# alanqrwang/keymorph

Hardware: AMD Instinct MI355X
Metric: volume-pairs/sec (fwd+bwd) at 256^3, 512 kp, TPS (higher is better)
Workload: dtype f32

## Files before the change

keymorph_amd/csrc/conv_up2.hip:

```cpp
#include <cstdlib>
#include "conv_split.h"

namespace {

constexpr int UX = 32, UY = 4;
constexpr int UHX = UX + 2, UHY = UY + 2, UPL = UHX * UHY * 3;
constexpr int UP_TPB = 512;
constexpr int UP_NST = 32;

template <int TERMS>
__global__ __launch_bounds__(256) void pack_weight_up_kernel(const float* __restrict__ w, __bf16* __restrict__ out,
                                                             int Cout, int Ctot, int cofs, int Cl, int CoutP, int nchunk,
                                                             const float* __restrict__ wscale) {
  const long long total = (long long)nchunk * UP_NST * 2 * CoutP * 8;
  for (long long e = (long long)blockIdx.x * 256 + threadIdx.x; e < total; e += (long long)gridDim.x * 256) {
    const int c = (int)(e & 7);
    long long r = e >> 3;
    const int col = (int)(r % CoutP); r /= CoutP;
    const int h = (int)(r & 1); r >>= 1;
    const int su = (int)(r % UP_NST);
    const int chunk = (int)(r / UP_NST);
    const int ci = chunk * 8 + c, p = su >> 2, st = su & 3;
    const int par[3] = {p >> 2, (p >> 1) & 1, p & 1}, j[3] = {st >> 1, st & 1, h};
    int lo[3], hi[3];
// ... 179 lines not shown
    long long r = e >> 3;
    const int col = (int)(r % CiP); r /= CiP;
    const int h = (int)(r & 1); r >>= 1;
    const int s = (int)(r % DUP_NST);
    const int chunk = (int)(r / DUP_NST);
    const int co = chunk * 8 + c;
    const int idx[3] = {s >> 3, (s >> 1) & 3, 2 * (s & 1) + h};
    int lo[3], hi[3];
#pragma unroll
    for (int a = 0; a < 3; ++a) {
      const int par = (idx[a] + 1) & 1, j = idx[a] <= 1 ? 1 : 0;
      lo[a] = par == 0 ? (j == 0 ? 0 : 1) : (j == 0 ? 0 : 2);
      hi[a] = par == 0 ? (j == 0 ? 0 : 2) : (j == 0 ? 1 : 2);
    }
    float v = 0.f;
    if (co < Cout && col < Cl) {
      const float* wr = w + ((long long)co * Ctot + cofs + col) * 27;
      for (int kz = lo[0]; kz <= hi[0]; ++kz)
        for (int ky = lo[1]; ky <= hi[1]; ++ky)
          for (int kx = lo[2]; kx <= hi[2]; ++kx) v += wr[kz * 9 + ky * 3 + kx];
    }
    float rem = wscale ? v * wscale[0] : v;
#pragma unroll
    for (int t = 0; t < TERMS; ++t) {
      float back;
      const unsigned short hb = to16<TERMS>(rem, back);
      reinterpret_cast<unsigned short*>(out)[((((long long)chunk * TERMS + t) * DUP_NST + s) * 2 + h) * CiP * 8 +
                                             (long long)col * 8 + c] = hb;
      rem -= back;
    }
  }
}

template <int TERMS, bool AMP = false>
__global__ __launch_bounds__(DUP_TPB, TERMS == 2 ? 2 : 3) void conv3_up2_dgrad_kernel(
    const float* __restrict__ dz , const bf16x8* __restrict__ wp,
    float* __restrict__ ds , int Dl, int Hl, int Wl, int Cl, int CiP, int Cout, int tiles_x,
    int tiles_y, const float* __restrict__ dscale, const float* __restrict__ wscale,
    double* __restrict__ stats_partial ,
    int in_blocked ) {
  __shared__ bf16x8 sIn[TERMS][DPL];
  const int tid = threadIdx.x, lane = tid & 63, wv = tid >> 6, li = lane & 31, lh = lane >> 5;
  const int n = blockIdx.z;
  const int ncig = (Cl + 127) / 128;
  const int item = xcd_remap(blockIdx.x, gridDim.x);
  const int cig = item % ncig, brick = item / ncig;
  const int bx = brick % tiles_x, by = (brick / tiles_x) % tiles_y, zl = brick / (tiles_x * tiles_y);
  const int x0 = bx * DUX, y0 = by * DUY;
  const int ci = cig * 128 + 32 * wv + li;
  const int D = 2 * Dl, H = 2 * Hl, W = 2 * Wl;

  f32x16 acc[2];
#pragma unroll
  for (int m = 0; m < 2; ++m)
#pragma unroll
    for (int r = 0; r < 16; ++r) acc[m][r] = 0.f;
  const float sD = dscale ? dscale[0] : 1.f;
  const float desc = (dscale ? dscale[1] : 1.f) * (wscale ? wscale[1] : 1.f);
  const int nchunk = (Cout + KC - 1) / KC;
  const float* dn = dz + (long long)n * D * H * W * Cout;
  constexpr int NV = (DPL + DUP_TPB - 1) / DUP_TPB;
  const int abase = (2 * (li >> 4)) * DHX + 2 * (li & 15) + lh;

  float4 pre[NV][2];
  auto fetch = [&](int ch) {
#pragma unroll
    for (int i = 0; i < NV; ++i) {
      const int v = tid + i * DUP_TPB;
      pre[i][0] = pre[i][1] = make_float4(0.f, 0.f, 0.f, 0.f);
      if (v < DPL) {
        const int lx = v % DHX, ly = (v / DHX) % DHY, lz = v / (DHX * DHY);
        const int gx = 2 * x0 - 1 + lx, gy = 2 * y0 - 1 + ly, gz = 2 * zl - 1 + lz;
        if ((unsigned)gx < (unsigned)W && (unsigned)gy < (unsigned)H && (unsigned)gz < (unsigned)D) {
          const long long vox = ((long long)gz * H + gy) * W + gx;
          const float* p = in_blocked ? dn + ((long long)ch * D * H * W + vox) * KC : dn + vox * Cout + ch * KC;
          if ((Cout & 3) == 0) {
#pragma unroll
            for (int q = 0; q < 2; ++q)
              if (ch * KC + 4 * q < Cout) pre[i][q] = *reinterpret_cast<const float4*>(p + 4 * q);
          } else {
            float t8[8] = {0.f, 0.f, 0.f, 0.f, 0.f, 0.f, 0.f, 0.f};
#pragma unroll
            for (int j = 0; j < 8; ++j)
              if (ch * KC + j < Cout) t8[j] = p[j];
            pre[i][0] = make_float4(t8[0], t8[1], t8[2], t8[3]);
            pre[i][1] = make_float4(t8[4], t8[5], t8[6], t8[7]);
          }
        }
      }
    }
  };
  constexpr bool PF = TERMS == 2;
  if (PF) fetch(0);
  for (int ch = 0; ch < nchunk; ++ch) {
    __syncthreads();
    if (!PF) fetch(ch);
#pragma unroll
    for (int i = 0; i < NV; ++i) {
      const int v = tid + i * DUP_TPB;
      if (v < DPL) {
        const float val[8] = {pre[i][0].x * sD, pre[i][0].y * sD, pre[i][0].z * sD, pre[i][0].w * sD,
                              pre[i][1].x * sD, pre[i][1].y * sD, pre[i][1].z * sD, pre[i][1].w * sD};
        bf16x8 parts[TERMS];
        split8<TERMS>(val, parts);
#pragma unroll
        for (int t = 0; t < TERMS; ++t) sIn[t][v] = parts[t];
      }
    }
    __syncthreads();
    if (PF && ch + 1 < nchunk) fetch(ch + 1);
    const bf16x8* wc = wp + (long long)ch * TERMS * DUP_NST * 2 * CiP + lh * CiP + ci;
    constexpr int BD = 4;
    bf16x8 bq[BD][TERMS];
#pragma unroll
    for (int d = 0; d < BD; ++d)
#pragma unroll
      for (int q = 0; q < TERMS; ++q) bq[d][q] = wc[((long long)(q * DUP_NST + d)) * 2 * CiP];
#pragma unroll 1
    for (int tz = 0; tz < 4; ++tz) {
#pragma unroll
      for (int s8 = 0; s8 < 8; ++s8) {
        const int s = tz * 8 + s8;
        bf16x8 b[TERMS];
#pragma unroll
        for (int q = 0; q < TERMS; ++q) b[q] = bq[s8 % BD][q];
        if (s + BD < DUP_NST) {
#pragma unroll
          for (int q = 0; q < TERMS; ++q) bq[s8 % BD][q] = wc[((long long)(q * DUP_NST + s + BD)) * 2 * CiP];
        }
        const int off = abase + (tz * DHY + (s8 >> 1)) * DHX + 2 * (s8 & 1);
#pragma unroll
        for (int m = 0; m < 2; ++m) {
          bf16x8 a[TERMS];
#pragma unroll
          for (int q = 0; q < TERMS; ++q) a[q] = sIn[q][off + 4 * m * DHX];
          if (TERMS == 3) {
            acc[m] = mfma16<TERMS>(a[2], b[0], acc[m]);
            acc[m] = mfma16<TERMS>(a[1], b[1], acc[m]);
            acc[m] = mfma16<TERMS>(a[0], b[2], acc[m]);
          }
          if constexpr (!AMP) {
            acc[m] = mfma16<TERMS>(a[1], b[0], acc[m]);
            acc[m] = mfma16<TERMS>(a[0], b[1], acc[m]);
          }
          acc[m] = mfma16<TERMS>(a[0], b[0], acc[m]);
        }
      }
    }
  }
  if (ci >= Cl) return;
  float s1 = 0.f, s2 = 0.f;
#pragma unroll
  for (int m = 0; m < 2; ++m) {
#pragma unroll
    for (int r = 0; r < 16; ++r) {
      const int row = (r & 3) + 8 * (r >> 2) + 4 * lh;
      const int gx = x0 + (row & 15), gy = y0 + 2 * m + (row >> 4);
      if (gx < Wl && gy < Hl) {
        const float v = acc[m][r] * desc;
        ds[((((long long)n * Dl + zl) * Hl + gy) * Wl + gx) * Cl + ci] = v;
        s1 += v;
        s2 = fmaf(v, v, s2);
      }
    }
  }
  if (stats_partial) {
    double d1 = (double)s1, d2 = (double)s2;
    d1 += __shfl_xor(d1, 32, 64);
    d2 += __shfl_xor(d2, 32, 64);
    if (lh == 0) {
      double* o = stats_partial + (((long long)n * gridDim.x / ncig + brick) * Cl + ci) * 2;
      o[0] = d1; o[1] = d2;
    }
  }
}

constexpr int GK = 32;
constexpr int GPITCH = GK * 2 + 16;
template <int TERMS, bool AMP = false>
__global__ __launch_bounds__(256, 3) void up2_wgrad_gemm_kernel(const float* __restrict__ A, const float* __restrict__ B,
                                                                float* __restrict__ Cp, int V, int Cl, int J, int kslab,
                                                                int ntn, int ntm, const float* __restrict__ ascale,
                                                                const float* __restrict__ bscale,
                                                                const float* __restrict__ a_scale ,
                                                                const float* __restrict__ a_shift, int xcd) {
  __shared__ __attribute__((aligned(16))) unsigned char sA[TERMS][128 * GPITCH];
  __shared__ __attribute__((aligned(16))) unsigned char sB[TERMS][128 * GPITCH];
  const int tid = threadIdx.x, lane = tid & 63, wv = tid >> 6, li = lane & 31, lh = lane >> 5;
  const int n = blockIdx.z;
  int item = xcd ? xcd_remap((int)blockIdx.x, (int)gridDim.x) : (int)blockIdx.x;
  const int tn = item % ntn; item /= ntn;
  const int tm = item % ntm;
  const int slab = item / ntm;
  const int m0 = tm * 128, n0 = tn * 128;
  const int wm = wv & 1, wn = wv >> 1;
  const float sa = ascale ? ascale[0] : 1.f, sb = bscale ? bscale[0] : 1.f;
  const float desc = (ascale ? ascale[1] : 1.f) * (bscale ? bscale[1] : 1.f);
  const float* An = A + (long long)n * V * Cl;
  const float* Bn = B + (long long)n * V * J;
  f32x16 acc[2][2];
#pragma unroll
  for (int i = 0; i < 2; ++i)
#pragma unroll
    for (int j = 0; j < 2; ++j)
#pragma unroll
// ... 455 lines not shown
  const int xcd = up2_xcd();
  const float* zero16 = (const float*)((const char*)ws + up2_fold_slab_bytes(N, Dl, Hl, Wl, Cl, Cout));
  if (hipMemsetAsync((void*)zero16, 0, 256, s) != hipSuccess) return -12;
  const bool amp = kmh_amp_enabled();
  int rc;
#define KMH_FOLD(A, M) launch_up2_fold<A, M>(g, s, xl, dz, (float*)ws, Dl, Hl, Wl, Cl, Cout, kt, tps, ntm, nto, ascale, dscale, \
                                             a_scale, a_shift, dz_blocked, xcd, zero16)
  if (mode == 2) rc = amp ? KMH_FOLD(true, 2) : KMH_FOLD(false, 2);
  else if (mode == 1) rc = amp ? KMH_FOLD(true, 1) : KMH_FOLD(false, 1);
  else rc = amp ? KMH_FOLD(true, 0) : KMH_FOLD(false, 0);
#undef KMH_FOLD
  if (rc) return rc;
  return up2_reduce(ws, ns, (long long)Cl * 27 * Cout, C, N, s);
}

KMH_API size_t kmh_conv3d_up2_dgrad_pack_bytes(int Cout, int Cl, int terms) {
  const int CiP = (Cl + 127) & ~127;
  return (size_t)((Cout + 7) / 8) * terms * DUP_NST * 2 * CiP * 8 * sizeof(__bf16);
}

KMH_API int kmh_conv3d_up2_dgrad_pack_weight(const float* w, void* packed, int Cout, int Ctot, int cofs, int Cl, int terms,
                                             const float* wscale, void* stream) {
  if (cofs < 0 || cofs + Cl > Ctot || (terms != 2 && terms != 3) || (terms == 2 && !wscale)) return -22;
  const int CiP = (Cl + 127) & ~127, nchunk = (Cout + 7) / 8;
  const long long total = (long long)nchunk * DUP_NST * 2 * CiP * 8;
  int nb = ceil_div(total, 256);
  if (nb > 2048) nb = 2048;
  hipStream_t s = (hipStream_t)stream;
  if (terms == 2) pack_weight_upt_kernel<2><<<nb, 256, 0, s>>>(w, (__bf16*)packed, Cout, Ctot, cofs, Cl, CiP, nchunk, wscale);
  else pack_weight_upt_kernel<3><<<nb, 256, 0, s>>>(w, (__bf16*)packed, Cout, Ctot, cofs, Cl, CiP, nchunk, wscale);
  return KMH_LAUNCH_CHECK();
}

KMH_API size_t kmh_conv3d_up2_dgrad_stats_ws_bytes(int N, int Dl, int Hl, int Wl, int Cl) {
  return (size_t)N * ceil_div(Wl, DUX) * ceil_div(Hl, DUY) * Dl * Cl * 2 * sizeof(double);
}
KMH_API int kmh_conv3d_up2_dgrad(const float* dz, const void* packed, float* ds, int N, int Dl, int Hl, int Wl, int Cl,
                                 int Cout, int terms, const float* dscale, const float* wscale, void* stats_ws,
                                 double* stats_out, int in_blocked, void* stream) {
  KmhAmpCall amp_call(terms);
  if ((terms != 2 && terms != 3) || (terms == 2 && (!dscale || !wscale)) || (stats_out && !stats_ws)) return -22;
  if (in_blocked && (Cout & 7)) return -22;
  const int CiP = (Cl + 127) & ~127;
  const int tx = ceil_div(Wl, DUX), ty = ceil_div(Hl, DUY);
  dim3 g(tx * ty * Dl * ceil_div(Cl, 128), 1, N);
  hipStream_t s = (hipStream_t)stream;
  double* sp = stats_out ? (double*)stats_ws : nullptr;
  if (terms == 2)
    if (kmh_amp_enabled())
      conv3_up2_dgrad_kernel<2, true><<<g, DUP_TPB, 0, s>>>(dz, (const bf16x8*)packed, ds, Dl, Hl, Wl, Cl, CiP, Cout, tx, ty, dscale, wscale, sp, in_blocked);
    else
    conv3_up2_dgrad_kernel<2><<<g, DUP_TPB, 0, s>>>(dz, (const bf16x8*)packed, ds, Dl, Hl, Wl, Cl, CiP, Cout, tx, ty, dscale, wscale, sp, in_blocked);
  else
    conv3_up2_dgrad_kernel<3><<<g, DUP_TPB, 0, s>>>(dz, (const bf16x8*)packed, ds, Dl, Hl, Wl, Cl, CiP, Cout, tx, ty, dscale, wscale, sp, in_blocked);
  if (stats_out)
    kmh_stats::final_kernel<<<dim3(ceil_div(Cl * 2, 256 / kWave), N), 256, 0, s>>>(sp, tx * ty * Dl, Cl, stats_out);
  return KMH_LAUNCH_CHECK();
}

KMH_API size_t kmh_conv3d_up2_pack_bytes(int Cout, int Cl, int terms) {
  return (size_t)(Cl / 8) * terms * UP_NST * 2 * cout_pad(Cout) * 8 * sizeof(__bf16);
}

KMH_API int kmh_conv3d_up2_pack_weight(const float* w, void* packed, int Cout, int Ctot, int cofs, int Cl, int terms,
                                       const float* wscale, void* stream) {
  if ((Cl & 7) || cofs < 0 || cofs + Cl > Ctot || (terms != 2 && terms != 3) || (terms == 2 && !wscale)) return -22;
  const int CoutP = cout_pad(Cout), nchunk = Cl / 8;
  const long long total = (long long)nchunk * UP_NST * 2 * CoutP * 8;
  int nb = ceil_div(total, 256);
  if (nb > 2048) nb = 2048;
  hipStream_t s = (hipStream_t)stream;
  if (terms == 2) pack_weight_up_kernel<2><<<nb, 256, 0, s>>>(w, (__bf16*)packed, Cout, Ctot, cofs, Cl, CoutP, nchunk, wscale);
  else pack_weight_up_kernel<3><<<nb, 256, 0, s>>>(w, (__bf16*)packed, Cout, Ctot, cofs, Cl, CoutP, nchunk, wscale);
  return KMH_LAUNCH_CHECK();
}

KMH_API int kmh_conv3d_up2_fwd(const float* xl, const float* scale, const float* shift, int Ctot, int cofs,
                               const void* packed, float* y, int N, int Dl, int Hl, int Wl, int Cl, int Cout, int terms,
                               const float* ascale, const float* wscale, void* stream) {
  KmhAmpCall amp_call(terms);
  if ((Cl & 7) || (terms != 2 && terms != 3) || (terms == 2 && (!ascale || !wscale))) return -22;
  if ((long long)Dl * Hl * Wl * Cl >= (1ll << 31)) return -22;
  const int CoutP = cout_pad(Cout);
  const int tx = ceil_div(Wl, UX), ty = ceil_div(Hl, UY);
  dim3 g(tx * ty * Dl * ceil_div(Cout, 64), 1, N);
  hipStream_t s = (hipStream_t)stream;
  if (terms == 2)
// ... 12 lines not shown
```

include/keymorph_hip.h:

```cpp
#ifndef KEYMORPH_HIP_H
#define KEYMORPH_HIP_H
#include <stddef.h>
#include <stdint.h>
#ifdef __cplusplus
extern "C" {
#endif

#define KMH_EINVAL (-22)
#define KMH_ABI_VERSION 1
int kmh_abi_version(void);

int kmh_grid_sample3d_fwd(const float* x, const float* grid, float* out, int N, int C, int D, int H,
                          int W, int Do, int Ho, int Wo, int mode, void* stream);
int kmh_grid_sample3d_bwd_grid(const float* x, const float* grid, const float* gout, float* dgrid,
                               int N, int C, int D, int H, int W, int Do, int Ho, int Wo, void* stream);
int kmh_grid_sample3d_bwd_input(const float* grid, const float* gout, float* dx, int N, int C, int D,
                                int H, int W, int Do, int Ho, int Wo, void* stream);

size_t kmh_reduce_ws_bytes(void);
int kmh_mse_fwd(const float* a, const float* b, long long n, float* out, void* ws, void* stream);
int kmh_mse_bwd(const float* a, const float* b, const float* gscale, long long n, float* da, void* stream);
int kmh_warp_mse_fwd(const float* x, const float* grid, const float* fixed, float* out, float* out_loss,
                     int N, int C, int D, int H, int W, int Do, int Ho, int Wo, void* ws, void* stream);
int kmh_warp_mse_fwd_grad(const float* x, const float* grid, const float* fixed, float* out, float* out_loss,
// ... 76 lines not shown
                  void* stream);
int kmh_com3d_bwd(const float* dpts, const float* feat, const float* sums, float* dfeat, int N, int K,
                  int D, int H, int W, void* stream);



int kmh_conv3d_pack_weight(const float* w, float* packed, int Cout, int Cin, int transposed, void* stream);
int kmh_conv3d_fwd(const float* x, const float* scale, const float* shift, const float* mask,
                   const float* packed_w, const float* bias, float* y, int N, int D, int H, int W, int Cin,
                   int Cout, int relu_in, int relu_out, void* stream);
size_t kmh_conv3d_pack_bf_bytes(int Cout, int Cin, int transposed, int terms);
int kmh_conv3d_pack_weight_bf(const float* w, void* packed, int Cout, int Cin, int transposed, int terms,
                              const float* wscale, void* stream);
size_t kmh_conv3d_fwd_bf_stats_ws_bytes(int N, int D, int H, int W, int Cout, int rows_per_wave);
int kmh_conv3d_fwd_bf(const float* x, const float* scale, const float* shift, const float* mask, const void* packed,
                      const float* bias, float* y, int N, int D, int H, int W, int Cin, int Cout, int relu_in,
                      int relu_out, int terms, int rows_per_wave, const float* ascale, const float* wscale,
                      void* stats_ws, double* stats_out, int in_blocked, const float* addend, void* stream);
int kmh_conv3d_fwd_bf_set_dispatch(int mode);
int kmh_conv3d_fwd_bf_split_ok(int N, int D, int H, int W, int Cin, int Cout, int terms);
int kmh_conv3d_fwd_bf_variant(int N, int D, int H, int W, int Cin, int Cout, int terms, int has_mask, int has_addend);
int kmh_conv3d_fwd_bf_pool_ok(int N, int D, int H, int W, int Cin, int Cout, int terms);
int kmh_conv3d_fwd_bf_pool(const float* x, const float* scale, const float* shift, const void* packed, float* yp,
                           unsigned char* arg, int N, int D, int H, int W, int Cin, int Cout, int relu_in, int terms,
                           const float* ascale, const float* wscale, void* stats_ws, double* stats_out, int in_blocked,
                           void* stream);
size_t kmh_conv3d_up2_pack_bytes(int Cout, int Cl, int terms);
int kmh_conv3d_up2_pack_weight(const float* w, void* packed, int Cout, int Ctot, int cofs, int Cl, int terms,
                               const float* wscale, void* stream);
size_t kmh_conv3d_up2_dgrad_pack_bytes(int Cout, int Cl, int terms);
int kmh_conv3d_up2_dgrad_pack_weight(const float* w, void* packed, int Cout, int Ctot, int cofs, int Cl, int terms,
                                     const float* wscale, void* stream);
size_t kmh_conv3d_up2_dgrad_stats_ws_bytes(int N, int Dl, int Hl, int Wl, int Cl);
int kmh_conv3d_up2_dgrad(const float* dz, const void* packed, float* ds, int N, int Dl, int Hl, int Wl, int Cl, int Cout,
                         int terms, const float* dscale, const float* wscale, void* stats_ws, double* stats_out,
                         int in_blocked ,
                         void* stream);
int kmh_up2_boxsum(const float* dz, float* G, int N, int Dl, int Hl, int Wl, int Cout, int in_blocked ,
                   void* stream);
size_t kmh_up2_wgrad_gemm_ws_bytes(int N, int V, int Cl, int J);
int kmh_up2_wgrad_gemm(const float* A, const float* B, float* C, int N, int V, int Cl, int J, int terms,
                       const float* ascale, const float* bscale, const float* a_scale, const float* a_shift, void* ws,
                       void* stream);
int kmh_up2_wgrad_fold_ok(int Cl, int Cout, int terms);
size_t kmh_up2_wgrad_fold_ws_bytes(int N, int Dl, int Hl, int Wl, int Cl, int Cout);
int kmh_up2_wgrad_fold(const float* xl, const float* dz, float* C, int N, int Dl, int Hl, int Wl, int Cl, int Cout, int terms,
                       const float* ascale, const float* dscale, const float* a_scale, const float* a_shift, int dz_blocked,
                       void* ws, void* stream);
int kmh_conv3d_up2_fwd(const float* xl, const float* scale, const float* shift, int Ctot, int cofs, const void* packed,
                       float* y, int N, int Dl, int Hl, int Wl, int Cl, int Cout, int terms, const float* ascale,
                       const float* wscale, void* stream);
size_t kmh_conv3d_wgrad_bf_ws_bytes(int N, int D, int H, int W, int Cin, int Cout, int terms);
int kmh_conv3d_wgrad_bf_blocked_ok(int N, int D, int H, int W, int Cin, int Cout, int terms);
int kmh_conv3d_wgrad_bf(const float* x, const float* scale, const float* shift, const float* dz,
                        const float* dzmask, float* dw, int N, int D, int H, int W, int Cin, int Cout, int relu_in,
                        int accumulate, int terms, int append_ones, const float* xscale, const float* dscale, int dz_blocked, const float* w_fold, double* bhat,
                        void* ws, void* stream);
size_t kmh_conv3d_first_layer_fwd_ws_bytes(int N, int D, int H, int W, int Cout);
int kmh_conv3d_first_layer_fwd(const float* x, const float* scale, const float* shift, const float* w, float* y, int N,
                               int D, int H, int W, int Cout, void* ws, double* stats_out, void* stream);
size_t kmh_conv3d_first_layer_wgrad_ws_bytes(int N, int D, int H, int W, int Cout);
int kmh_conv3d_first_layer_wgrad(const float* x, const float* dz, const float* dzmask, const float* c123, double* rs, int N,
                                 int D, int H, int W, int Cout, void* ws, void* stream);
int kmh_conv3d_first_layer_fold(const void* rs, int rs_f64, const float* w, const float* scale_n, const float* shift_n, int Cout,
                                float* dw, double* ab_n, int accumulate, void* stream);
size_t kmh_conv3d_wgrad_ws_bytes(int N, int D, int H, int W, int Cin, int Cout);
// ... 78 lines not shown
```

keymorph_amd/_lib.py:

```python
from __future__ import annotations

import ctypes as C
import os

from .build import LIBPATH

_f = C.c_void_p
_i = C.c_int
_ll = C.c_longlong
_sz = C.c_size_t

PROTOS = {
    "kmh_abi_version": (_i, []),
    "kmh_grid_sample3d_fwd": (_i, [_f, _f, _f, _i, _i, _i, _i, _i, _i, _i, _i, _i, _f]),
    "kmh_grid_sample3d_bwd_grid": (_i, [_f, _f, _f, _f, _i, _i, _i, _i, _i, _i, _i, _i, _f]),
    "kmh_grid_sample3d_bwd_input": (_i, [_f, _f, _f, _i, _i, _i, _i, _i, _i, _i, _i, _f]),
    "kmh_reduce_ws_bytes": (_sz, []),
    "kmh_mse_fwd": (_i, [_f, _f, _ll, _f, _f, _f]),
    "kmh_mse_bwd": (_i, [_f, _f, _f, _ll, _f, _f]),
    "kmh_warp_mse_fwd": (_i, [_f, _f, _f, _f, _f, _i, _i, _i, _i, _i, _i, _i, _i, _f, _f]),
    "kmh_warp_mse_fwd_grad": (_i, [_f, _f, _f, _f, _f, _f, _i, _i, _i, _i, _i, _i, _i, _i, _f, _f]),
    "kmh_scale_unless_one": (_i, [_f, _ll, _f, _f]),
    "kmh_dice_sums": (_i, [_f, _f, _i, _ll, _f, _f, _f]),
    "kmh_rows_axpby": (_i, [_f, _f, _f, _f, _i, _ll, _f, _f]),
# ... 19 lines not shown
    "kmh_rigid_fit_fwd": (_i, [_f, _f, _f, _f, _i, _i, _f]),
    "kmh_rigid_fit_bwd": (_i, [_f, _f, _f, _f, _f, _f, _f, _i, _i, _f]),
    "kmh_affine_inverse_fwd": (_i, [_f, _f, _i, _f]),
    "kmh_affine_inverse_bwd": (_i, [_f, _f, _f, _i, _f]),
    "kmh_affine_points_fwd": (_i, [_f, _f, _f, _i, _i, _f]),
    "kmh_jacobian_det": (_i, [_f, _ll, _ll, _i, _i, _i, _f, _f, _f, _f]),
    "kmh_label_presence": (_i, [_f, _ll, _i, _f, _f]),
    "kmh_one_hot_select": (_i, [_f, _i, _ll, _f, _i, _f, _i, _f]),
    "kmh_hausdorff3d_ws_bytes": (_sz, [_i, _i, _i]),
    "kmh_hausdorff3d": (_i, [_f, _f, _i, _i, _ll, _ll, _i, _i, _i, _i, C.c_double, C.c_double, C.c_double, _f, _f, _f]),
    "kmh_edt3d_sq_ws_bytes": (_sz, [_i, _i, _i]),
    "kmh_edt3d_sq": (_i, [_f, _i, _i, _i, _i, C.c_double, C.c_double, C.c_double, _f, _f, _f]),
    "kmh_label_counts": (_i, [_f, _f, _i, _i, _i, _ll, _f, _f]),
    "kmh_lc2_ws_bytes": (_sz, [_i, _i]),
    "kmh_lc2_fwd": (_i, [_f, _f, _i, _i, _i, _f, _i, C.c_double, C.c_double, _i, _f, _f, _f]),
    "kmh_lc2_bwd": (_i, [_f, _f, _f, _i, _i, _i, _f, _i, _i, _f, _f, _f, _f]),
    "kmh_affine_build_matrix": (_i, [_f, _f, _f, _f, _f, _i, _f]),
    "kmh_affine_points_bwd": (_i, [_f, _f, _f, _f, _f, _i, _i, _f]),
    "kmh_com3d_fwd": (_i, [_f, _f, _f, _i, _i, _i, _i, _i, _f, _f]),
    "kmh_com3d_bwd": (_i, [_f, _f, _f, _f, _i, _i, _i, _i, _i, _f]),
    "kmh_conv3d_pack_weight": (_i, [_f, _f, _i, _i, _i, _f]),
    "kmh_conv3d_fwd": (_i, [_f, _f, _f, _f, _f, _f, _f, _i, _i, _i, _i, _i, _i, _i, _i, _f]),
    "kmh_conv3d_pack_bf_bytes": (_sz, [_i, _i, _i, _i]),
    "kmh_conv3d_pack_weight_bf": (_i, [_f, _f, _i, _i, _i, _i, _f, _f]),
    "kmh_conv3d_fwd_bf": (_i, [_f, _f, _f, _f, _f, _f, _f, _i, _i, _i, _i, _i, _i, _i, _i, _i, _i, _f, _f, _f, _f, _i, _f, _f]),
    "kmh_conv3d_fwd_bf_set_dispatch": (_i, [_i]),
    "kmh_conv3d_fwd_bf_variant": (_i, [_i, _i, _i, _i, _i, _i, _i, _i, _i]),
    "kmh_conv3d_fwd_bf_pool_ok": (_i, [_i, _i, _i, _i, _i, _i, _i]),
    "kmh_conv3d_fwd_bf_split_ok": (_i, [_i, _i, _i, _i, _i, _i, _i]),
    "kmh_conv3d_fwd_bf_pool": (_i, [_f, _f, _f, _f, _f, _f, _i, _i, _i, _i, _i, _i, _i, _i, _f, _f, _f, _f, _i, _f]),
    "kmh_conv3d_up2_dgrad_pack_bytes": (_sz, [_i, _i, _i]),
    "kmh_conv3d_up2_dgrad_pack_weight": (_i, [_f, _f, _i, _i, _i, _i, _i, _f, _f]),
    "kmh_conv3d_up2_dgrad_stats_ws_bytes": (_sz, [_i, _i, _i, _i, _i]),
    "kmh_conv3d_up2_dgrad": (_i, [_f, _f, _f, _i, _i, _i, _i, _i, _i, _i, _f, _f, _f, _f, _i, _f]),
    "kmh_up2_boxsum": (_i, [_f, _f, _i, _i, _i, _i, _i, _i, _f]),
    "kmh_up2_wgrad_gemm_ws_bytes": (_sz, [_i, _i, _i, _i]),
    "kmh_up2_wgrad_gemm": (_i, [_f, _f, _f, _i, _i, _i, _i, _i, _f, _f, _f, _f, _f, _f]),
    "kmh_up2_wgrad_fold_ok": (_i, [_i, _i, _i]),
    "kmh_up2_wgrad_fold_ws_bytes": (_sz, [_i, _i, _i, _i, _i, _i]),
    "kmh_up2_wgrad_fold": (_i, [_f, _f, _f, _i, _i, _i, _i, _i, _i, _i, _f, _f, _f, _f, _i, _f, _f]),
    "kmh_conv3d_up2_pack_bytes": (_sz, [_i, _i, _i]),
    "kmh_conv3d_up2_pack_weight": (_i, [_f, _f, _i, _i, _i, _i, _i, _f, _f]),
    "kmh_conv3d_up2_fwd": (_i, [_f, _f, _f, _i, _i, _f, _f, _i, _i, _i, _i, _i, _i, _i, _f, _f, _f]),
    "kmh_conv3d_fwd_bf_stats_ws_bytes": (_sz, [_i, _i, _i, _i, _i, _i]),
    "kmh_conv3d_first_layer_fwd_ws_bytes": (_sz, [_i, _i, _i, _i, _i]),
    "kmh_conv3d_first_layer_fwd": (_i, [_f, _f, _f, _f, _f, _i, _i, _i, _i, _i, _f, _f, _f]),
    "kmh_conv3d_wgrad_bf_ws_bytes": (_sz, [_i, _i, _i, _i, _i, _i, _i]),
    "kmh_conv3d_wgrad_bf": (_i, [_f, _f, _f, _f, _f, _f, _i, _i, _i, _i, _i, _i, _i, _i, _i, _i, _f, _f, _i, _f, _f, _f, _f]),
    "kmh_conv3d_wgrad_bf_blocked_ok": (_i, [_i, _i, _i, _i, _i, _i, _i]),
    "kmh_conv3d_first_layer_wgrad_ws_bytes": (_sz, [_i, _i, _i, _i, _i]),
    "kmh_conv3d_first_layer_wgrad": (_i, [_f, _f, _f, _f, _f, _i, _i, _i, _i, _i, _f, _f]),
    "kmh_conv3d_first_layer_fold": (_i, [_f, _i, _f, _f, _f, _i, _f, _f, _i, _f]),
    "kmh_conv3d_wgrad_ws_bytes": (_sz, [_i, _i, _i, _i, _i, _i]),
    "kmh_conv3d_wgrad": (_i, [_f, _f, _f, _f, _f, _f, _i, _i, _i, _i, _i, _i, _i, _i, _f, _f]),
    "kmh_channel_stats_ws_bytes": (_sz, [_i, _i]),
    "kmh_channel_stats": (_i, [_f, _f, _i, _i, _ll, _i, _f, _f, _f, _f]),
    "kmh_gn_fwd_coeffs": (_i, [_f, _f, _f, _i, _i, _i, C.c_double, C.c_float, _f, _f, _f, _f, _f]),
    "kmh_absmax_scale": (_i, [_f, _ll, C.c_float, _f, _f]),
    "kmh_gn_bwd_coeffs": (_i, [_f, _f, _f, _i, _i, _i, C.c_double, _f, _f, _f, _f, _f]),
    "kmh_gn_bwd_coeffs_fold": (_i, [_f, _f, _f, _f, _f, _i, _i, _i, C.c_double, _f, _f, _f, _f, _f]),
    "kmh_gn_bwd_apply": (_i, [_f, _f, _f, _i, _ll, _i, _i, _i, _f, _f, _i, _f]),
    "kmh_in_bwd_stats": (_i, [_f, _f, _f, _f, _i, _ll, _i, _f, _f, _f]),
    "kmh_in_bwd_apply": (_i, [_f, _f, _f, _f, _f, _i, _ll, _i, _f, _f, _f]),
    "kmh_in_bwd_apply_pool": (_i, [_f, _f, _f, _f, _f, _f, _i, _i, _i, _i, _i, _f, _f, _f]),
    "kmh_relu_mask": (_i, [_f, _f, _ll, _f, _f]),
    "kmh_norm_apply": (_i, [_f, _f, _f, _i, _ll, _i, _i, _f, _f]),
# ... 124 lines not shown
```

keymorph_amd/backbone_ops.py:

```python
from __future__ import annotations

import os
from typing import Optional, Tuple

import torch

from . import _lib
from ._handoff import attach, expect, peek
from ._lib import check
from .ops import _p, _prep, _stream, workspace

Tensor = torch.Tensor
EPS = 1e-5

CONV_MODE = os.environ.get("KEYMORPH_HIP_CONV", "f16x3")
_TERMS = {"f16x3": 2, "bf16x6": 3}
_HEAD_TERMS = {"f16x3": 2, "bf16x6": 3}
BF_ROWS_PER_WAVE = int(os.environ.get("KEYMORPH_HIP_BF_ROWS", "4"))


def set_conv_mode(mode: str):
    global CONV_MODE
    assert mode in ("f32", "f16x3", "bf16x6"), mode
    CONV_MODE = mode


_SWITCHES = {
    "KEYMORPH_NO_EPILOGUE_STATS": "a separate statistics pass per layer instead of the convolution epilogue's",
    "KEYMORPH_NO_UPCONV": "materialise upsample+concat instead of the fused decoder operator, forward",
    "KEYMORPH_NO_UPCONV_BWD": "materialise upsample+concat instead of the fused decoder operator, backward",
    "KEYMORPH_NO_UPCONV_WGRAD": "the fused decoder operator rebuilds the upsampled half for the 27-tap weight gradient",
    "KEYMORPH_NO_UP2_FOLD": "the upsampled channels' weight gradient by the box-sum tensor + matrix product route",
    "KEYMORPH_NO_STATS_FOLD": "GroupNorm's backward statistics by a pass over the tensors",
    "KEYMORPH_NO_BLOCKED_GRADS": "every gradient in (N,D,H,W,C)",
    "KEYMORPH_NO_BLOCKED_UPCAT": "only the fused decoder operator's gradient in (N,D,H,W,C)",
    "KEYMORPH_NO_SPLIT_POOLGRAD": "the 256^3-level pooled gradient scattered as fp32 instead of pre-split records",
    "KEYMORPH_NO_CONV_POOL": "separate pooling pass instead of the conv epilogue's",
    "KEYMORPH_NO_LAZY_FIRST": "GroupNorm backward of the first block as its own pass",
    "KEYMORPH_NO_LAZY_SKIP": "GroupNorm's backward of a decoder skip applied in the decoder",
    "KEYMORPH_NO_LAZY_IN": "ConvNet block by block: separate norm / ReLU / pooling passes",
    "KEYMORPH_RANGE_AUDIT": "debug (ON = audit): per-sample dynamic range of every gradient operand, RANGE_AUDIT_LOG",
}


def _off(name: str) -> bool:
    if name not in _SWITCHES:
        raise KeyError(name)
    return bool(os.environ.get(name))


import contextlib
import functools
import threading

_AMP_DEFAULT = os.environ.get("KEYMORPH_AMP", "0") not in ("", "0")
_amp_tls = threading.local()


def amp_enabled() -> bool:
    return bool(getattr(_amp_tls, "on", _AMP_DEFAULT))


@contextlib.contextmanager
def amp_scope(on: bool):
    prev = amp_enabled()
# ... 269 lines not shown
        xscale = absmax_scale(x, 1.0) if terms == 2 else None
        dscale = (dscale if dscale is not None else absmax_scale(dy)) if terms == 2 else None
        for n in range(N):
            if _lib.profiler.enabled:
                _lib.profiler.meta = {"flops": 2.0 * 27 * 1 * Cout * V, "shape": (1, D, H, W, 1, Cout)}
            check(lib.kmh_conv3d_wgrad_bf(_p(x[n]), None, None, _p(dy[n]), _p(None if ymask is None else ymask[n]),
                                          _p(rs), 1, D, H, W, 2, Cout, 0, 0, _t(terms), 1, _p(xscale), _p(dscale), 0, None, None,
                                          _p(ws), _stream()), "kmh_conv3d_wgrad_bf")
            check(lib.kmh_conv3d_first_layer_fold(_p(rs), 0, _p(weight), _p(scale[n]), _p(shift[n]), Cout, _p(dw),
                                                  _p(ab[n]), int(n > 0), _stream()), "kmh_conv3d_first_layer_fold")
    _, dgamma, dbeta = _gn_bwd_coeffs(ab, gamma, mr, N, 1, G, V)
    return dw, dgamma, dbeta


def conv3_up2_dgrad(dz: Tensor, weight: Tensor, Cs: int, Cl: int, dscale: Optional[Tensor] = None,
                    stats_out: Optional[Tensor] = None, dz_blocked: bool = False) -> Tensor:
    lib = _lib.load()
    N, D, H, W, Cout = dz.shape
    terms = _TERMS[CONV_MODE]
    wsu = None
    if terms == 2:
        wsu = absmax_scale(weight[:, Cs:].contiguous()) * _const(dz.device, 0.125, 8.0)
        if dscale is None:
            dscale = absmax_scale(dz)
    pk = torch.empty(int(lib.kmh_conv3d_up2_dgrad_pack_bytes(Cout, Cl, terms)), dtype=torch.uint8, device=dz.device)
    check(lib.kmh_conv3d_up2_dgrad_pack_weight(_p(weight), _p(pk), Cout, Cs + Cl, Cs, Cl, terms, _p(wsu), _stream()),
          "kmh_conv3d_up2_dgrad_pack_weight")
    ds = _f32((N, D // 2, H // 2, W // 2, Cl), dz.device)
    _conv_meta(N, D, H, W, Cout, Cl, taps=8)
    sws = None
    if stats_out is not None:
        sws = workspace(int(lib.kmh_conv3d_up2_dgrad_stats_ws_bytes(N, D // 2, H // 2, W // 2, Cl)), dz.device, "convstats")
    check(lib.kmh_conv3d_up2_dgrad(_p(dz), _p(pk), _p(ds), N, D // 2, H // 2, W // 2, Cl, Cout, _t(terms),
                                   _p(dscale if terms == 2 else None), _p(wsu), _p(sws), _p(stats_out), int(dz_blocked),
                                   _stream()), "kmh_conv3d_up2_dgrad")
    return ds


UPCONV_STATS = {"calls": 0}


def _up_sources(x):
    tag = peek(x, "up_sources")
    return tag[:2] if (tag is not None and tag[0]._version == tag[2] and tag[1]._version == tag[3]) else None


def grad_blocked_ok(N, D, H, W, Cin, Cout) -> bool:
    if CONV_MODE != "f16x3" or _off("KEYMORPH_NO_BLOCKED_GRADS"):
        return False
    return bool(_lib.load().kmh_conv3d_wgrad_bf_blocked_ok(N, D, H, W, Cin, Cout, 2))


BLOCKED_STATS = {"handoffs": 0}
SPLIT_STATS = {"handoffs": 0}


UP2_STATS = {"fold": 0, "boxsum": 0}


def up2_wgrad_fold_ok(Cl, Cout, terms):
    if _off("KEYMORPH_NO_UP2_FOLD"):
        return False
    return bool(_lib.load().kmh_up2_wgrad_fold_ok(int(Cl), int(Cout), int(terms)))


def pool_grad_split_ok(N, D, H, W, Cin, Cout) -> bool:
    if CONV_MODE != "f16x3" or _off("KEYMORPH_NO_SPLIT_POOLGRAD") or Cout % 8:
        return False
# ... 888 lines not shown
```

Before: 15.78.

## Block two z-slices per up2 dgrad workgroup with split-x LDS layout

The up2 dgrad kernel can now compute ZB=2 output z-slices per workgroup. The staged halo grows from 4 to 6 fine z-planes, and each weight fetch feeds twice as many MFMA tiles, which cuts weight loads and halo re-reads per output. For the ZB=2 path the LDS image is stored with even and odd x split into two halves (row pitch 40), likely to avoid bank conflicts. LDS moves to dynamic shared memory set with hipFuncSetAttribute, and the stats slab indexing is recomputed per slice. The cost is more accumulator registers, a smaller weight prefetch depth, and launch bounds fixed at 2 for all variants.

```diff
diff --git a/keymorph_amd/csrc/conv_up2.hip b/keymorph_amd/csrc/conv_up2.hip
--- a/keymorph_amd/csrc/conv_up2.hip
+++ b/keymorph_amd/csrc/conv_up2.hip
@@ -235,35 +235,55 @@
   }
 }
 
-template <int TERMS, bool AMP = false>
-__global__ __launch_bounds__(DUP_TPB, TERMS == 2 ? 2 : 3) void conv3_up2_dgrad_kernel(
+#ifndef KMH_DG_SPLITX
+#define KMH_DG_SPLITX 1
+#endif
+template <int ZB>
+struct DgradGeom {
+  static constexpr bool SPLITX = ZB == 2 && KMH_DG_SPLITX;
+  static constexpr int NZ = 2 * ZB + 2;
+  static constexpr int HXH = DUX + 1;
+  static constexpr int PX = SPLITX ? 40 : DHX;
+  static constexpr int NVOX = DHX * DHY * NZ;
+  static constexpr int IMG = PX * DHY * NZ;
+  static constexpr int MT = 2 * ZB;
+};
+template <int TERMS, int ZB>
+constexpr int up2_dgrad_lds_bytes() { return TERMS * DgradGeom<ZB>::IMG * 16; }
+
+template <int TERMS, bool AMP = false, int ZB = 1>
+__global__ __launch_bounds__(DUP_TPB, 2) void conv3_up2_dgrad_kernel(
     const float* __restrict__ dz , const bf16x8* __restrict__ wp,
     float* __restrict__ ds , int Dl, int Hl, int Wl, int Cl, int CiP, int Cout, int tiles_x,
     int tiles_y, const float* __restrict__ dscale, const float* __restrict__ wscale,
     double* __restrict__ stats_partial ,
     int in_blocked ) {
-  __shared__ bf16x8 sIn[TERMS][DPL];
+  using G = DgradGeom<ZB>;
+  constexpr int DPLV = G::NVOX, PX = G::PX, MT = G::MT;
+  constexpr bool SPLITX = G::SPLITX;
+  extern __shared__ __attribute__((aligned(16))) unsigned char up2d_lds[];
+  bf16x8* sIn = reinterpret_cast<bf16x8*>(up2d_lds);
   const int tid = threadIdx.x, lane = tid & 63, wv = tid >> 6, li = lane & 31, lh = lane >> 5;
   const int n = blockIdx.z;
   const int ncig = (Cl + 127) / 128;
   const int item = xcd_remap(blockIdx.x, gridDim.x);
   const int cig = item % ncig, brick = item / ncig;
-  const int bx = brick % tiles_x, by = (brick / tiles_x) % tiles_y, zl = brick / (tiles_x * tiles_y);
+  const int bx = brick % tiles_x, by = (brick / tiles_x) % tiles_y, zl = ZB * (brick / (tiles_x * tiles_y));
   const int x0 = bx * DUX, y0 = by * DUY;
   const int ci = cig * 128 + 32 * wv + li;
   const int D = 2 * Dl, H = 2 * Hl, W = 2 * Wl;
 
-  f32x16 acc[2];
-#pragma unroll
-  for (int m = 0; m < 2; ++m)
+  f32x16 acc[MT];
+#pragma unroll
+  for (int m = 0; m < MT; ++m)
 #pragma unroll
     for (int r = 0; r < 16; ++r) acc[m][r] = 0.f;
   const float sD = dscale ? dscale[0] : 1.f;
   const float desc = (dscale ? dscale[1] : 1.f) * (wscale ? wscale[1] : 1.f);
   const int nchunk = (Cout + KC - 1) / KC;
   const float* dn = dz + (long long)n * D * H * W * Cout;
-  constexpr int NV = (DPL + DUP_TPB - 1) / DUP_TPB;
-  const int abase = (2 * (li >> 4)) * DHX + 2 * (li & 15) + lh;
+  constexpr int NV = (DPLV + DUP_TPB - 1) / DUP_TPB;
+  const int abase = SPLITX ? (2 * (li >> 4)) * PX + lh * G::HXH + (li & 15) : (2 * (li >> 4)) * PX + 2 * (li & 15) + lh;
 
   float4 pre[NV][2];
   auto fetch = [&](int ch) {
@@ -271,7 +291,7 @@
     for (int i = 0; i < NV; ++i) {
       const int v = tid + i * DUP_TPB;
       pre[i][0] = pre[i][1] = make_float4(0.f, 0.f, 0.f, 0.f);
-      if (v < DPL) {
+      if (v < DPLV) {
         const int lx = v % DHX, ly = (v / DHX) % DHY, lz = v / (DHX * DHY);
         const int gx = 2 * x0 - 1 + lx, gy = 2 * y0 - 1 + ly, gz = 2 * zl - 1 + lz;
         if ((unsigned)gx < (unsigned)W && (unsigned)gy < (unsigned)H && (unsigned)gz < (unsigned)D) {
@@ -301,19 +321,24 @@
 #pragma unroll
     for (int i = 0; i < NV; ++i) {
       const int v = tid + i * DUP_TPB;
-      if (v < DPL) {
+      if (v < DPLV) {
         const float val[8] = {pre[i][0].x * sD, pre[i][0].y * sD, pre[i][0].z * sD, pre[i][0].w * sD,
                               pre[i][1].x * sD, pre[i][1].y * sD, pre[i][1].z * sD, pre[i][1].w * sD};
         bf16x8 parts[TERMS];
         split8<TERMS>(val, parts);
-#pragma unroll
-        for (int t = 0; t < TERMS; ++t) sIn[t][v] = parts[t];
+        int slot = v;
+        if constexpr (SPLITX) {
+          const int lx = v % DHX, row = v / DHX;
+          slot = row * PX + (lx & 1) * G::HXH + (lx >> 1);
+        }
+#pragma unroll
+        for (int t = 0; t < TERMS; ++t) sIn[t * G::IMG + slot] = parts[t];
       }
     }
     __syncthreads();
     if (PF && ch + 1 < nchunk) fetch(ch + 1);
     const bf16x8* wc = wp + (long long)ch * TERMS * DUP_NST * 2 * CiP + lh * CiP + ci;
-    constexpr int BD = 4;
+    constexpr int BD = ZB == 2 ? 2 : 4;
     bf16x8 bq[BD][TERMS];
 #pragma unroll
     for (int d = 0; d < BD; ++d)
@@ -331,12 +356,12 @@
 #pragma unroll
           for (int q = 0; q < TERMS; ++q) bq[s8 % BD][q] = wc[((long long)(q * DUP_NST + s + BD)) * 2 * CiP];
         }
-        const int off = abase + (tz * DHY + (s8 >> 1)) * DHX + 2 * (s8 & 1);
-#pragma unroll
-        for (int m = 0; m < 2; ++m) {
+        const int off = abase + (tz * DHY + (s8 >> 1)) * PX + (SPLITX ? 1 : 2) * (s8 & 1);
+#pragma unroll
+        for (int m = 0; m < MT; ++m) {
           bf16x8 a[TERMS];
 #pragma unroll
-          for (int q = 0; q < TERMS; ++q) a[q] = sIn[q][off + 4 * m * DHX];
+          for (int q = 0; q < TERMS; ++q) a[q] = sIn[q * G::IMG + off + (2 * (m >> 1) * DHY + 4 * (m & 1)) * PX];
           if (TERMS == 3) {
             acc[m] = mfma16<TERMS>(a[2], b[0], acc[m]);
             acc[m] = mfma16<TERMS>(a[1], b[1], acc[m]);
@@ -352,28 +377,33 @@
     }
   }
   if (ci >= Cl) return;
-  float s1 = 0.f, s2 = 0.f;
-#pragma unroll
-  for (int m = 0; m < 2; ++m) {
-#pragma unroll
-    for (int r = 0; r < 16; ++r) {
-      const int row = (r & 3) + 8 * (r >> 2) + 4 * lh;
-      const int gx = x0 + (row & 15), gy = y0 + 2 * m + (row >> 4);
-      if (gx < Wl && gy < Hl) {
-        const float v = acc[m][r] * desc;
-        ds[((((long long)n * Dl + zl) * Hl + gy) * Wl + gx) * Cl + ci] = v;
-        s1 += v;
-        s2 = fmaf(v, v, s2);
-      }
-    }
-  }
-  if (stats_partial) {
-    double d1 = (double)s1, d2 = (double)s2;
-    d1 += __shfl_xor(d1, 32, 64);
-    d2 += __shfl_xor(d2, 32, 64);
-    if (lh == 0) {
-      double* o = stats_partial + (((long long)n * gridDim.x / ncig + brick) * Cl + ci) * 2;
-      o[0] = d1; o[1] = d2;
+#pragma unroll
+  for (int zs = 0; zs < ZB; ++zs) {
+    if (zl + zs >= Dl) break;
+    float s1 = 0.f, s2 = 0.f;
+#pragma unroll
+    for (int m = 0; m < 2; ++m) {
+#pragma unroll
+      for (int r = 0; r < 16; ++r) {
+        const int row = (r & 3) + 8 * (r >> 2) + 4 * lh;
+        const int gx = x0 + (row & 15), gy = y0 + 2 * m + (row >> 4);
+        if (gx < Wl && gy < Hl) {
+          const float v = acc[2 * zs + m][r] * desc;
+          ds[((((long long)n * Dl + zl + zs) * Hl + gy) * Wl + gx) * Cl + ci] = v;
+          s1 += v;
+          s2 = fmaf(v, v, s2);
+        }
+      }
+    }
+    if (stats_partial) {
+      double d1 = (double)s1, d2 = (double)s2;
+      d1 += __shfl_xor(d1, 32, 64);
+      d2 += __shfl_xor(d2, 32, 64);
+      if (lh == 0) {
+        const long long slab = (long long)(zl + zs) * tiles_y * tiles_x + by * tiles_x + bx;
+        double* o = stats_partial + (((long long)n * tiles_x * tiles_y * Dl + slab) * Cl + ci) * 2;
+        o[0] = d1; o[1] = d2;
+      }
     }
   }
 }
@@ -895,6 +925,20 @@
   return KMH_LAUNCH_CHECK();
 }
 
+static int up2_legacy() { const char* e = getenv("KEYMORPH_UP2_LEGACY"); return e && atoi(e) != 0; }
+
+template <int TERMS, bool AMP, int ZB>
+static int launch_up2_dgrad(hipStream_t s, int N, const float* dz, const void* packed, float* ds, int Dl, int Hl, int Wl, int Cl, int CiP,
+                            int Cout, int tx, int ty, const float* dscale, const float* wscale, double* sp, int in_blocked) {
+  constexpr int lds = up2_dgrad_lds_bytes<TERMS, ZB>();
+  hipError_t e = hipFuncSetAttribute((const void*)conv3_up2_dgrad_kernel<TERMS, AMP, ZB>, hipFuncAttributeMaxDynamicSharedMemorySize, lds);
+  if (e != hipSuccess) return (int)e;
+  dim3 g(tx * ty * ceil_div(Dl, ZB) * ceil_div(Cl, 128), 1, N);
+  conv3_up2_dgrad_kernel<TERMS, AMP, ZB><<<g, DUP_TPB, lds, s>>>(dz, (const bf16x8*)packed, ds, Dl, Hl, Wl, Cl, CiP, Cout, tx, ty, dscale,
+                                                                wscale, sp, in_blocked);
+  return 0;
+}
+
 KMH_API size_t kmh_conv3d_up2_dgrad_stats_ws_bytes(int N, int Dl, int Hl, int Wl, int Cl) {
   return (size_t)N * ceil_div(Wl, DUX) * ceil_div(Hl, DUY) * Dl * Cl * 2 * sizeof(double);
 }
@@ -906,16 +950,16 @@
   if (in_blocked && (Cout & 7)) return -22;
   const int CiP = (Cl + 127) & ~127;
   const int tx = ceil_div(Wl, DUX), ty = ceil_div(Hl, DUY);
-  dim3 g(tx * ty * Dl * ceil_div(Cl, 128), 1, N);
   hipStream_t s = (hipStream_t)stream;
   double* sp = stats_out ? (double*)stats_ws : nullptr;
-  if (terms == 2)
-    if (kmh_amp_enabled())
-      conv3_up2_dgrad_kernel<2, true><<<g, DUP_TPB, 0, s>>>(dz, (const bf16x8*)packed, ds, Dl, Hl, Wl, Cl, CiP, Cout, tx, ty, dscale, wscale, sp, in_blocked);
-    else
-    conv3_up2_dgrad_kernel<2><<<g, DUP_TPB, 0, s>>>(dz, (const bf16x8*)packed, ds, Dl, Hl, Wl, Cl, CiP, Cout, tx, ty, dscale, wscale, sp, in_blocked);
-  else
-    conv3_up2_dgrad_kernel<3><<<g, DUP_TPB, 0, s>>>(dz, (const bf16x8*)packed, ds, Dl, Hl, Wl, Cl, CiP, Cout, tx, ty, dscale, wscale, sp, in_blocked);
+  const bool amp = kmh_amp_enabled(), two = terms == 2 && !up2_legacy();
+  int rc;
+#define KMH_DG(T, A, ZB) launch_up2_dgrad<T, A, ZB>(s, N, dz, packed, ds, Dl, Hl, Wl, Cl, CiP, Cout, tx, ty, dscale, wscale, sp, in_blocked)
+  if (terms == 3) rc = KMH_DG(3, false, 1);
+  else if (amp) rc = two ? KMH_DG(2, true, 2) : KMH_DG(2, true, 1);
+  else rc = two ? KMH_DG(2, false, 2) : KMH_DG(2, false, 1);
+#undef KMH_DG
+  if (rc) return rc;
   if (stats_out)
     kmh_stats::final_kernel<<<dim3(ceil_div(Cl * 2, 256 / kWave), N), 256, 0, s>>>(sp, tx * ty * Dl, Cl, stats_out);
   return KMH_LAUNCH_CHECK();
```

Result: no change. 15.93 (median of 6 runs) (+1.0%).

## Add two-plane brick kernel for decoder upsample data-gradient

Applied to the files above, without the earlier changes.

Adds a new up2 dgrad kernel in which each block covers two low-resolution depth planes. It stages a six-plane high-resolution halo in shared memory and accumulates both output planes in one set of MFMA accumulators. This halves the block count and reuses the overlapping dz halo and weight loads across the two planes, cutting global and LDS traffic. The cost is more registers per thread (launch bounds of 2), a larger shared-memory footprint, and a scheduling barrier. An env flag falls back to the one-plane kernel, and the stats layout keeps one record per plane.

```diff
diff --git a/include/keymorph_hip.h b/include/keymorph_hip.h
--- a/include/keymorph_hip.h
+++ b/include/keymorph_hip.h
@@ -132,6 +132,7 @@
 int kmh_conv3d_up2_dgrad_pack_weight(const float* w, void* packed, int Cout, int Ctot, int cofs, int Cl, int terms,
                                      const float* wscale, void* stream);
 size_t kmh_conv3d_up2_dgrad_stats_ws_bytes(int N, int Dl, int Hl, int Wl, int Cl);
+int kmh_conv3d_up2_dgrad_brick_planes(int terms, int in_blocked);
 int kmh_conv3d_up2_dgrad(const float* dz, const void* packed, float* ds, int N, int Dl, int Hl, int Wl, int Cl, int Cout,
                          int terms, const float* dscale, const float* wscale, void* stats_ws, double* stats_out,
                          int in_blocked ,
diff --git a/keymorph_amd/_lib.py b/keymorph_amd/_lib.py
--- a/keymorph_amd/_lib.py
+++ b/keymorph_amd/_lib.py
@@ -75,6 +75,7 @@
     "kmh_conv3d_up2_dgrad_pack_bytes": (_sz, [_i, _i, _i]),
     "kmh_conv3d_up2_dgrad_pack_weight": (_i, [_f, _f, _i, _i, _i, _i, _i, _f, _f]),
     "kmh_conv3d_up2_dgrad_stats_ws_bytes": (_sz, [_i, _i, _i, _i, _i]),
+    "kmh_conv3d_up2_dgrad_brick_planes": (_i, [_i, _i]),
     "kmh_conv3d_up2_dgrad": (_i, [_f, _f, _f, _i, _i, _i, _i, _i, _i, _i, _f, _f, _f, _f, _i, _f]),
     "kmh_up2_boxsum": (_i, [_f, _f, _i, _i, _i, _i, _i, _i, _f]),
     "kmh_up2_wgrad_gemm_ws_bytes": (_sz, [_i, _i, _i, _i]),
diff --git a/keymorph_amd/backbone_ops.py b/keymorph_amd/backbone_ops.py
--- a/keymorph_amd/backbone_ops.py
+++ b/keymorph_amd/backbone_ops.py
@@ -31,6 +31,7 @@
     "KEYMORPH_NO_UPCONV_BWD": "materialise upsample+concat instead of the fused decoder operator, backward",
     "KEYMORPH_NO_UPCONV_WGRAD": "the fused decoder operator rebuilds the upsampled half for the 27-tap weight gradient",
     "KEYMORPH_NO_UP2_FOLD": "the upsampled channels' weight gradient by the box-sum tensor + matrix product route",
+    "KEYMORPH_NO_UP2_DGRAD_Z2": "the decoder's low-resolution data gradient over one-plane bricks (the kernel the two-plane one replaced)",
     "KEYMORPH_NO_STATS_FOLD": "GroupNorm's backward statistics by a pass over the tensors",
     "KEYMORPH_NO_BLOCKED_GRADS": "every gradient in (N,D,H,W,C)",
     "KEYMORPH_NO_BLOCKED_UPCAT": "only the fused decoder operator's gradient in (N,D,H,W,C)",
@@ -366,8 +367,9 @@
     if stats_out is not None:
         sws = workspace(int(lib.kmh_conv3d_up2_dgrad_stats_ws_bytes(N, D // 2, H // 2, W // 2, Cl)), dz.device, "convstats")
     check(lib.kmh_conv3d_up2_dgrad(_p(dz), _p(pk), _p(ds), N, D // 2, H // 2, W // 2, Cl, Cout, _t(terms),
-                                   _p(dscale if terms == 2 else None), _p(wsu), _p(sws), _p(stats_out), int(dz_blocked),
-                                   _stream()), "kmh_conv3d_up2_dgrad")
+                                   _p(dscale if terms == 2 else None), _p(wsu), _p(sws), _p(stats_out),
+                                   int(dz_blocked) | (2 if _off("KEYMORPH_NO_UP2_DGRAD_Z2") else 0), _stream()),
+          "kmh_conv3d_up2_dgrad")
     return ds
 
 
diff --git a/keymorph_amd/csrc/conv_up2.hip b/keymorph_amd/csrc/conv_up2.hip
--- a/keymorph_amd/csrc/conv_up2.hip
+++ b/keymorph_amd/csrc/conv_up2.hip
@@ -374,6 +374,167 @@
     if (lh == 0) {
       double* o = stats_partial + (((long long)n * gridDim.x / ncig + brick) * Cl + ci) * 2;
       o[0] = d1; o[1] = d2;
+    }
+  }
+}
+
+constexpr int D2HZ = 6;
+constexpr int D2_VOX = DHX * DHY * D2HZ;
+constexpr int D2_HXP = DHX / 2;
+constexpr int D2_RT = 2 * DHY, D2_RP = 2 * D2_RT, D2_RZ = 2 * D2_RP;
+constexpr int D2_SLOTS = 3 * D2_RZ * D2_HXP;
+#ifndef KMH_D2_SB
+#define KMH_D2_SB 1
+#endif
+
+template <bool AMP>
+__global__ __launch_bounds__(DUP_TPB, 2) void conv3_up2_dgrad_z2_kernel(
+    const float* __restrict__ dz, const bf16x8* __restrict__ wp, float* __restrict__ ds, int Dl, int Hl, int Wl, int Cl, int CiP,
+    int Cout, int tiles_x, int tiles_y, const float* __restrict__ dscale, const float* __restrict__ wscale,
+    double* __restrict__ stats_partial , int in_blocked) {
+  __shared__ bf16x8 sIn[D2_SLOTS];
+  const int tid = threadIdx.x, lane = tid & 63, wv = tid >> 6, li = lane & 31, lh = lane >> 5;
+  const int n = blockIdx.z;
+  const int ncig = (Cl + 127) / 128;
+  const int item = xcd_remap(blockIdx.x, gridDim.x);
+  const int cig = item % ncig, brick = item / ncig;
+  const int bx = brick % tiles_x, by = (brick / tiles_x) % tiles_y, z0 = 2 * (brick / (tiles_x * tiles_y));
+  const int x0 = bx * DUX, y0 = by * DUY;
+  const int ci = cig * 128 + 32 * wv + li;
+  const int D = 2 * Dl, H = 2 * Hl, W = 2 * Wl;
+
+  f32x16 acc[4];
+#pragma unroll
+  for (int m = 0; m < 4; ++m)
+#pragma unroll
+    for (int r = 0; r < 16; ++r) acc[m][r] = 0.f;
+  const float sD = dscale ? dscale[0] : 1.f;
+  const float desc = (dscale ? dscale[1] : 1.f) * (wscale ? wscale[1] : 1.f);
+  const int nchunk = (Cout + KC - 1) / KC;
+  const float* dn = dz + (long long)n * D * H * W * Cout;
+  constexpr int NV = (D2_VOX + DUP_TPB - 1) / DUP_TPB;
+  const int abase = ((li >> 4) * D2_RZ + lh * D2_RP) * D2_HXP + (li & 15);
+  const unsigned wlane = (unsigned)(lh * CiP + ci) * (unsigned)sizeof(bf16x8);
+
+  float4 pre[NV][2];
+  auto fetch = [&](int ch) {
+#pragma unroll
+    for (int i = 0; i < NV; ++i) {
+      const int v = tid + i * DUP_TPB;
+      pre[i][0] = pre[i][1] = make_float4(0.f, 0.f, 0.f, 0.f);
+      if (v < D2_VOX) {
+        const int lx = v % DHX, ly = (v / DHX) % DHY, lz = v / (DHX * DHY);
+        const int gx = 2 * x0 - 1 + lx, gy = 2 * y0 - 1 + ly, gz = 2 * z0 - 1 + lz;
+        if ((unsigned)gx < (unsigned)W && (unsigned)gy < (unsigned)H && (unsigned)gz < (unsigned)D) {
+          const long long vox = ((long long)gz * H + gy) * W + gx;
+          const float* p = in_blocked ? dn + ((long long)ch * D * H * W + vox) * KC : dn + vox * Cout + ch * KC;
+          if ((Cout & 3) == 0) {
+#pragma unroll
+            for (int q = 0; q < 2; ++q)
+              if (ch * KC + 4 * q < Cout) pre[i][q] = *reinterpret_cast<const float4*>(p + 4 * q);
+          } else {
+            float t8[8] = {0.f, 0.f, 0.f, 0.f, 0.f, 0.f, 0.f, 0.f};
+#pragma unroll
+            for (int j = 0; j < 8; ++j)
+              if (ch * KC + j < Cout) t8[j] = p[j];
+            pre[i][0] = make_float4(t8[0], t8[1], t8[2], t8[3]);
+            pre[i][1] = make_float4(t8[4], t8[5], t8[6], t8[7]);
+          }
+        }
+      }
+    }
+  };
+  auto commit = [&]() {
+#pragma unroll
+    for (int i = 0; i < NV; ++i) {
+      const int v = tid + i * DUP_TPB;
+      if (v < D2_VOX) {
+        const int lx = v % DHX, ly = (v / DHX) % DHY, lz = v / (DHX * DHY);
+        const float val[8] = {pre[i][0].x * sD, pre[i][0].y * sD, pre[i][0].z * sD, pre[i][0].w * sD,
+                              pre[i][1].x * sD, pre[i][1].y * sD, pre[i][1].z * sD, pre[i][1].w * sD};
+        bf16x8 parts[2];
+        split8<2>(val, parts);
+        const int slot = ((lz >> 1) * D2_RZ + (lx & 1) * D2_RP + (lz & 1) * DHY + ly) * D2_HXP + (lx >> 1);
+#pragma unroll
+        for (int t = 0; t < 2; ++t) sIn[slot + t * D2_RT * D2_HXP] = parts[t];
+      }
+    }
+  };
+  fetch(0);
+  for (int ch = 0; ch < nchunk; ++ch) {
+    __syncthreads();
+    commit();
+    __syncthreads();
+    if (ch + 1 < nchunk) fetch(ch + 1);
+    const char* wc = reinterpret_cast<const char*>(wp + (long long)ch * 2 * DUP_NST * 2 * CiP);
+    auto wld = [&](int q, int s) {
+      return *reinterpret_cast<const bf16x8*>(wc + (long long)(q * DUP_NST + s) * 2 * CiP * (int)sizeof(bf16x8) + wlane);
+    };
+    constexpr int BD = 4;
+    bf16x8 bq[BD][2];
+#pragma unroll
+    for (int d = 0; d < BD; ++d)
+#pragma unroll
+      for (int q = 0; q < 2; ++q) bq[d][q] = wld(q, d);
+#pragma unroll 1
+    for (int tz = 0; tz < 4; ++tz) {
+      const int zbase = abase + ((tz >> 1) * D2_RZ + (tz & 1) * DHY) * D2_HXP;
+#pragma unroll
+      for (int s8 = 0; s8 < 8; ++s8) {
+        const int s = tz * 8 + s8;
+        bf16x8 b[2];
+#pragma unroll
+        for (int q = 0; q < 2; ++q) b[q] = bq[s8 % BD][q];
+        if (s + BD < DUP_NST) {
+#pragma unroll
+          for (int q = 0; q < 2; ++q) bq[s8 % BD][q] = wld(q, s + BD);
+        }
+        const int off = zbase + (s8 >> 1) * D2_HXP + (s8 & 1);
+#pragma unroll
+        for (int m = 0; m < 4; ++m) {
+          bf16x8 a[2];
+#pragma unroll
+          for (int q = 0; q < 2; ++q) a[q] = sIn[off + (q * D2_RT + 2 * m) * D2_HXP];
+          if constexpr (!AMP) {
+            acc[m] = mfma16<2>(a[1], b[0], acc[m]);
+            acc[m] = mfma16<2>(a[0], b[1], acc[m]);
+          }
+          acc[m] = mfma16<2>(a[0], b[0], acc[m]);
+        }
+#if KMH_D2_SB
+        __builtin_amdgcn_sched_barrier(0);
+#endif
+      }
+    }
+  }
+  if (ci >= Cl) return;
+#pragma unroll
+  for (int zp = 0; zp < 2; ++zp) {
+    const int zl = z0 + zp;
+    if (zl >= Dl) continue;
+    float s1 = 0.f, s2 = 0.f;
+#pragma unroll
+    for (int m = 0; m < 4; ++m) {
+#pragma unroll
+      for (int rr = 0; rr < 8; ++rr) {
+        const int gx = x0 + (rr & 3) + 8 * (rr >> 2) + 4 * lh, gy = y0 + m;
+        if (gx < Wl && gy < Hl) {
+          const float v = acc[m][8 * zp + rr] * desc;
+          ds[((((long long)n * Dl + zl) * Hl + gy) * Wl + gx) * Cl + ci] = v;
+          s1 += v;
+          s2 = fmaf(v, v, s2);
+        }
+      }
+    }
+    if (stats_partial) {
+      double d1 = (double)s1, d2 = (double)s2;
+      d1 += __shfl_xor(d1, 32, 64);
+      d2 += __shfl_xor(d2, 32, 64);
+      if (lh == 0) {
+        const long long rec = ((long long)n * Dl + zl) * tiles_y * tiles_x + by * tiles_x + bx;
+        double* o = stats_partial + (rec * Cl + ci) * 2;
+        o[0] = d1; o[1] = d2;
+      }
     }
   }
 }
@@ -898,18 +1059,28 @@
 KMH_API size_t kmh_conv3d_up2_dgrad_stats_ws_bytes(int N, int Dl, int Hl, int Wl, int Cl) {
   return (size_t)N * ceil_div(Wl, DUX) * ceil_div(Hl, DUY) * Dl * Cl * 2 * sizeof(double);
 }
+KMH_API int kmh_conv3d_up2_dgrad_brick_planes(int terms, int in_blocked) {
+  return (terms == 1 || terms == 2) && !(in_blocked & 2) ? 2 : 1;
+}
 KMH_API int kmh_conv3d_up2_dgrad(const float* dz, const void* packed, float* ds, int N, int Dl, int Hl, int Wl, int Cl,
                                  int Cout, int terms, const float* dscale, const float* wscale, void* stats_ws,
                                  double* stats_out, int in_blocked, void* stream) {
   KmhAmpCall amp_call(terms);
   if ((terms != 2 && terms != 3) || (terms == 2 && (!dscale || !wscale)) || (stats_out && !stats_ws)) return -22;
+  const bool z2 = kmh_conv3d_up2_dgrad_brick_planes(terms, in_blocked) == 2;
+  in_blocked &= 1;
   if (in_blocked && (Cout & 7)) return -22;
   const int CiP = (Cl + 127) & ~127;
   const int tx = ceil_div(Wl, DUX), ty = ceil_div(Hl, DUY);
-  dim3 g(tx * ty * Dl * ceil_div(Cl, 128), 1, N);
+  dim3 g(tx * ty * (z2 ? ceil_div(Dl, 2) : Dl) * ceil_div(Cl, 128), 1, N);
   hipStream_t s = (hipStream_t)stream;
   double* sp = stats_out ? (double*)stats_ws : nullptr;
-  if (terms == 2)
+  if (z2)
+    if (kmh_amp_enabled())
+      conv3_up2_dgrad_z2_kernel<true><<<g, DUP_TPB, 0, s>>>(dz, (const bf16x8*)packed, ds, Dl, Hl, Wl, Cl, CiP, Cout, tx, ty, dscale, wscale, sp, in_blocked);
+    else
+      conv3_up2_dgrad_z2_kernel<false><<<g, DUP_TPB, 0, s>>>(dz, (const bf16x8*)packed, ds, Dl, Hl, Wl, Cl, CiP, Cout, tx, ty, dscale, wscale, sp, in_blocked);
+  else if (terms == 2)
     if (kmh_amp_enabled())
       conv3_up2_dgrad_kernel<2, true><<<g, DUP_TPB, 0, s>>>(dz, (const bf16x8*)packed, ds, Dl, Hl, Wl, Cl, CiP, Cout, tx, ty, dscale, wscale, sp, in_blocked);
     else
```

New measurement: 15.59 before, 15.71 after, median of 6. Within noise of the previous version (+0.8%).
